# kkromberg/SpeechRecognition

Hardware: AMD Instinct MI355X
Metric: frames/sec scored+decoded (higher is better)
Workload: dtype f64

## Files before the change

include/srgpu.h:

```cpp
#ifndef SRGPU_H
#define SRGPU_H

#include <stddef.h>
#include <stdint.h>

#ifdef __cplusplus
extern "C" {
#endif

#if defined(__GNUC__)
#define SR_API __attribute__((visibility("default")))
#else
#define SR_API
#endif

#define SR_ABI_VERSION 4
SR_API int sr_abi_version(void);

#define SR_OK 0
#define SR_EINVAL (-1)
#define SR_EHIP (-2)
#define SR_ENODEV (-3)
#define SR_ELIMIT (-4)
#define SR_ENOMEM (-5)
// ... 205 lines not shown
                                         double* out_am);
SR_API int sr_bigram_lattice_nbest(uint32_t n_frames, uint64_t n_arcs, const uint32_t* word, const uint32_t* hist,
                                   const uint32_t* first, const uint32_t* last, const double* am, uint32_t n_words,
                                   uint32_t silence_word, const float* lm, double lm_scale, uint32_t n_best, uint32_t* out_words,
                                   uint64_t words_cap, uint64_t* out_off, double* out_cost, uint32_t* out_count);

typedef struct sr_bigram_stream sr_bigram_stream;
SR_API int sr_bigram_stream_open(sr_model* m, sr_bigram* b, const sr_bigram_params* p, uint32_t max_streams, uint64_t max_frames,
                                 sr_bigram_stream** out);
SR_API int sr_bigram_stream_begin(sr_bigram_stream* s, uint32_t* id);
SR_API int sr_bigram_stream_push(sr_bigram_stream* s, uint32_t n, const uint32_t* ids, const float* feats, const uint64_t* frame_off);
SR_API int sr_bigram_stream_partial(sr_bigram_stream* s, uint32_t id, uint32_t* out_word, float* out_score, uint32_t* out_time,
                                    uint32_t cap, uint32_t* count, uint64_t* frames);
SR_API int sr_bigram_stream_end(sr_bigram_stream* s, uint32_t id, uint32_t* out_word, float* out_score, uint32_t* out_time,
                                uint32_t cap, uint32_t* count);
SR_API int sr_bigram_stream_destroy(sr_bigram_stream* s);

SR_API int sr_probe_fp16_denormals(int device, int* preserved);
SR_API int sr_probe_fp16_accumulation(int device, int* within_model, double* worst_ratio);

typedef struct {
  double gmm_ms;
  uint64_t gmm_launches;
  double gmm_flops;
  double search_ms;
  uint64_t search_launches;
  double search_bytes;
  uint64_t frames;
  uint64_t refined_pairs;
  uint64_t refined_densities;
  double prefilter_ms;
  double refine_ms;
} sr_profile;
SR_API int sr_profile_enable(sr_model* m, int on);
SR_API int sr_profile_reset(sr_model* m);
SR_API int sr_profile_read(sr_model* m, sr_profile* out);

#ifdef __cplusplus
}
#endif
#endif
```

speechrecognition_amd/capi.py:

```python
from __future__ import annotations

import ctypes as C
import os

import numpy as np

HERE = os.path.dirname(os.path.abspath(__file__))
LIB_PATH = os.environ.get("SRGPU_LIB") or os.path.join(HERE, "libsrgpu.so")

GMM_MFMA, GMM_EXACT, GMM_PREFILTER, GMM_DEFAULT = 0, 1, 2, 3
POOL_GLOBAL, POOL_MIXTURE, POOL_NONE = 0, 1, 2
SEARCH_GENERAL_KERNEL = 1
SEARCH_SLOT_KERNEL = 2
BIGRAM_DENSE_STATES = 1
BIGRAM_GLOBAL_STATES = 2
SR_ECORRUPT = -7
SR_ABI_VERSION = 4

SYMBOLS = [
    "sr_abi_version", "sr_model_trim",
    "sr_last_error", "sr_device_count", "sr_model_create", "sr_model_load_mixset", "sr_model_destroy", "sr_model_info",
    "sr_corpus_upload", "sr_corpus_upload_async", "sr_corpus_wait", "sr_corpus_destroy", "sr_shard_utterances", "sr_recognize_batch_multi", "sr_score_corpus", "sr_score_frames", "sr_lexicon_create",
    "sr_lexicon_destroy", "sr_lexicon_describe", "sr_recognize_corpus", "sr_traceback_corpus", "sr_traceback_words", "sr_recognize_batch", "sr_align_corpus", "sr_align_corpus_pruned", "sr_path_scores_corpus", "sr_model_create_from_statistics", "sr_model_create_from_accumulated", "sr_mixset_write", "sr_model_set_tying", "sr_model_tying_info", "sr_model_topology", "sr_accumulate_corpus",
    "sr_state_posteriors_corpus", "sr_baum_welch_corpus", "sr_word_posteriors_corpus", "sr_recognize_confidence_corpus",
    "sr_net_occupancies_corpus", "sr_mmi_statistics_corpus", "sr_model_create_from_mmi_statistics",
    "sr_smbr_max_positions", "sr_net_accuracies_corpus", "sr_smbr_statistics_corpus",
    "sr_word_lattice_corpus", "sr_lattice_nbest",
    "sr_fmllr_statistics_corpus", "sr_fmllr_statistics_bw_corpus", "sr_fmllr_estimate", "sr_corpus_transform",
    "sr_bigram_create", "sr_bigram_destroy", "sr_bigram_describe", "sr_recognize_bigram_corpus",
    "sr_bigram_word_posteriors_corpus", "sr_recognize_bigram_confidence_corpus",
    "sr_bigram_occupancies_corpus", "sr_bigram_mmi_statistics_corpus",
    "sr_bigram_word_lattice_corpus", "sr_bigram_lattice_nbest",
    "sr_stream_open", "sr_stream_begin", "sr_stream_push", "sr_stream_partial", "sr_stream_end", "sr_stream_destroy",
    "sr_bigram_stream_open", "sr_bigram_stream_begin", "sr_bigram_stream_push", "sr_bigram_stream_partial", "sr_bigram_stream_end",
    "sr_bigram_stream_destroy",
    "sr_probe_fp16_denormals", "sr_probe_fp16_accumulation",
    "sr_profile_enable", "sr_profile_reset", "sr_profile_read",
]


class SrError(RuntimeError):
    def __init__(self, code, msg):
        super().__init__(f"libsrgpu error {code}: {msg}")
        self.code = code


def smbr_max_positions():
    n = C.c_uint32()
    _check(lib().sr_smbr_max_positions(C.byref(n)))
    return n.value


class SearchParams(C.Structure):
    _fields_ = [("am_threshold", C.c_double), ("word_penalty", C.c_double), ("gmm_kernel", C.c_int), ("flags", C.c_int)]


class BigramParams(C.Structure):
    _fields_ = [("acoustic_pruning", C.c_float), ("lm_pruning", C.c_float), ("gmm_kernel", C.c_int), ("max_word_ends", C.c_uint32), ("flags", C.c_int)]


class Profile(C.Structure):
    _fields_ = [("gmm_ms", C.c_double), ("gmm_launches", C.c_uint64), ("gmm_flops", C.c_double),
                ("search_ms", C.c_double), ("search_launches", C.c_uint64), ("search_bytes", C.c_double),
                ("frames", C.c_uint64), ("refined_pairs", C.c_uint64), ("refined_densities", C.c_uint64),
                ("prefilter_ms", C.c_double), ("refine_ms", C.c_double)]


_lib = None


# ... 48 lines not shown
        L.sr_recognize_confidence_corpus.argtypes = [vp, vp, vp, C.POINTER(SearchParams), dbl, vp, vp, vp, vp, vp]
        L.sr_net_occupancies_corpus.argtypes = [vp, vp, vp, C.POINTER(SearchParams), dbl, dbl, u32, vp, vp, vp, vp, vp, vp]
        L.sr_mmi_statistics_corpus.argtypes = [vp, vp, vp, C.POINTER(SearchParams), dbl, dbl, i32, vp, vp] + [vp] * 10
        L.sr_smbr_max_positions.argtypes = [vp]
        L.sr_net_accuracies_corpus.argtypes = [vp, vp, vp, C.POINTER(SearchParams), dbl, dbl, u32, vp, vp, vp, vp, vp, vp]
        L.sr_smbr_statistics_corpus.argtypes = [vp, vp, vp, C.POINTER(SearchParams), dbl, dbl, i32, vp] + [vp] * 10
        L.sr_model_create_from_mmi_statistics.argtypes = [vp] + [vp] * 8 + [dbl, dbl, dbl, C.POINTER(vp)]
        L.sr_word_lattice_corpus.argtypes = [vp, vp, vp, C.POINTER(SearchParams), dbl, u64, vp, vp, vp, vp, vp, vp, vp, vp]
        L.sr_lattice_nbest.argtypes = [u32, u64, vp, vp, vp, vp, u32, u32, vp, u64, vp, vp, C.POINTER(u32)]
        L.sr_bigram_create.argtypes = [vp, u32, vp, vp, u32, vp, vp, C.POINTER(vp)]
        L.sr_bigram_destroy.argtypes = [vp]
        L.sr_bigram_describe.argtypes = [vp, C.c_char_p, C.c_size_t]
        L.sr_recognize_bigram_corpus.argtypes = [vp, vp, vp, C.POINTER(BigramParams), vp, vp, vp, vp]
        L.sr_bigram_word_posteriors_corpus.argtypes = [vp, vp, vp, i32, dbl, dbl, u32, vp, vp, vp, vp]
        L.sr_bigram_occupancies_corpus.argtypes = [vp, vp, vp, i32, dbl, dbl, u32, vp, vp, vp, vp, vp, vp]
        L.sr_bigram_mmi_statistics_corpus.argtypes = [vp, vp, vp, i32, dbl, dbl, i32, vp, vp] + [vp] * 10
        L.sr_recognize_bigram_confidence_corpus.argtypes = [vp, vp, vp, C.POINTER(BigramParams), dbl, vp, vp, vp, vp, vp]
        L.sr_bigram_word_lattice_corpus.argtypes = [vp, vp, vp, i32, dbl, u64] + [vp] * 10
        L.sr_bigram_lattice_nbest.argtypes = [u32, u64, vp, vp, vp, vp, vp, u32, u32, vp, dbl, u32, vp, u64, vp, vp, C.POINTER(u32)]
        L.sr_stream_open.argtypes = [vp, vp, C.POINTER(SearchParams), u32, u64, C.POINTER(vp)]
        L.sr_stream_begin.argtypes = [vp, C.POINTER(u32)]
        L.sr_stream_push.argtypes = [vp, u32, vp, vp, vp]
        L.sr_stream_partial.argtypes = [vp, u32, vp, u32, C.POINTER(u32), C.POINTER(u64)]
        L.sr_stream_end.argtypes = [vp, u32, vp, u32, C.POINTER(u32), vp, vp, vp]
        L.sr_stream_destroy.argtypes = [vp]
        L.sr_bigram_stream_open.argtypes = [vp, vp, C.POINTER(BigramParams), u32, u64, C.POINTER(vp)]
        L.sr_bigram_stream_begin.argtypes = [vp, C.POINTER(u32)]
        L.sr_bigram_stream_push.argtypes = [vp, u32, vp, vp, vp]
        L.sr_bigram_stream_partial.argtypes = [vp, u32, vp, vp, vp, u32, C.POINTER(u32), C.POINTER(u64)]
        L.sr_bigram_stream_end.argtypes = [vp, u32, vp, vp, vp, u32, C.POINTER(u32)]
        L.sr_bigram_stream_destroy.argtypes = [vp]
        L.sr_probe_fp16_denormals.argtypes = [i32, C.POINTER(i32)]
        L.sr_probe_fp16_accumulation.argtypes = [i32, C.POINTER(i32), C.POINTER(dbl)]
        L.sr_profile_enable.argtypes = [vp, i32]
        L.sr_profile_reset.argtypes = [vp]
        L.sr_profile_read.argtypes = [vp, C.POINTER(Profile)]
        _lib = L
    return _lib


def _check(rc):
    if rc != 0:
        raise SrError(rc, lib().sr_last_error().decode(errors="replace"))


def device_count():
    n = C.c_int(0)
    _check(lib().sr_device_count(C.byref(n)))
    return n.value


def _ptr(a):
    return a.ctypes.data if a is not None else None


class Model:

    def __init__(self, handle):
        self.h = handle
        d, s, c = C.c_uint32(), C.c_uint32(), C.c_uint64()
        _check(lib().sr_model_info(self.h, C.byref(d), C.byref(s), C.byref(c)))
        self.dim, self.n_states, self.n_densities = d.value, s.value, c.value

    @classmethod
    def from_mixset(cls, path, dim, pooling=POOL_NONE, max_approx=True, device=0):
        h = C.c_void_p()
# ... 50 lines not shown
        self.close()

    def score_frames(self, feats, kernel=GMM_PREFILTER):
        feats = np.ascontiguousarray(feats, dtype=np.float32)
        out = np.empty((feats.shape[0], self.n_states), dtype=np.float64)
        _check(lib().sr_score_frames(self.h, _ptr(feats), feats.shape[0], kernel, _ptr(out)))
        return out

    def upload(self, feats, frame_off, asynchronous=False):
        return Corpus(self, feats, frame_off, asynchronous)

    def recognize_batch(self, lexicon, feats, frame_off, am_threshold, word_penalty, kernel=GMM_PREFILTER):
        feats = np.ascontiguousarray(feats, dtype=np.float32)
        frame_off = np.ascontiguousarray(frame_off, dtype=np.uint64)
        n = len(frame_off) - 1
        words = np.zeros(max(int(frame_off[-1]), 1), dtype=np.uint32)
        woff = np.zeros(n + 1, dtype=np.uint64)
        sp = SearchParams(am_threshold, word_penalty, kernel, 0)
        _check(lib().sr_recognize_batch(self.h, lexicon.h, C.byref(sp), _ptr(feats), _ptr(frame_off), n, _ptr(words), _ptr(woff)))
        return words[: int(woff[-1])].copy(), woff

    def lexicon(self, word_off, automaton, silence_idx, tdp, silence_state):
        return Lexicon(self, word_off, automaton, silence_idx, tdp, silence_state)

    def bigram(self, word_off, mixtures, silence_word, lm, tdp):
        return Bigram(self, word_off, mixtures, silence_word, lm, tdp)

    def stream(self, lexicon, am_threshold, word_penalty, kernel=GMM_PREFILTER, max_streams=1, max_frames=65535):
        return Stream(self, lexicon, am_threshold, word_penalty, kernel, max_streams, max_frames)

    def bigram_stream(self, bigram, acoustic_pruning=None, lm_pruning=None, kernel=GMM_PREFILTER, max_streams=1, max_frames=65535):
        return BigramStream(self, bigram, FLT_MAX if acoustic_pruning is None else acoustic_pruning,
                            FLT_MAX if lm_pruning is None else lm_pruning, kernel, max_streams, max_frames)

    def profile(self, on=True):
        _check(lib().sr_profile_enable(self.h, int(on)))
        _check(lib().sr_profile_reset(self.h))

    def profile_read(self):
        p = Profile()
        _check(lib().sr_profile_read(self.h, C.byref(p)))
        return {k: getattr(p, k) for k, _ in Profile._fields_}


FLT_MAX = float(np.finfo(np.float32).max)


class Bigram:

    def __init__(self, model, word_off, mixtures, silence_word, lm, tdp):
        self.model = model
        word_off = np.ascontiguousarray(word_off, dtype=np.uint32)
        mixtures = np.ascontiguousarray(mixtures, dtype=np.uint16)
        W = len(word_off) - 1
        lm = np.ascontiguousarray(lm, dtype=np.float32)
        assert lm.shape == (W, W)
        tdp = np.ascontiguousarray(tdp, dtype=np.float32)
        assert tdp.size == 8
        self.h = C.c_void_p()
        _check(lib().sr_bigram_create(model.h, W, _ptr(word_off), _ptr(mixtures), silence_word, _ptr(lm), _ptr(tdp), C.byref(self.h)))

    def describe(self):
        buf = C.create_string_buffer(32)
        _check(lib().sr_bigram_describe(self.h, buf, len(buf)))
        return buf.value.decode()

# ... 545 lines not shown
```

speechrecognition_amd/csrc/gmm_prefilter.hip:

```cpp
#include <hip/hip_runtime.h>
#include <stdint.h>

#include <algorithm>
#include <cmath>
#include <vector>

#include "kernels.h"

#ifndef SR_P16_NB
#define SR_P16_NB 4
#endif

namespace srgpu {

typedef float v4f __attribute__((ext_vector_type(4)));
static constexpr int kPWaves = 4;
static constexpr int kGroupBlocks = 8;

typedef _Float16 f16x8 __attribute__((ext_vector_type(8)));

__device__ inline uint32_t pack_f16x2(_Float16 l, _Float16 h) {
  return (uint32_t)__builtin_bit_cast(uint16_t, l) | ((uint32_t)__builtin_bit_cast(uint16_t, h) << 16);
}

// ... 286 lines not shown
  switch (ks32) {
    case 1: hipLaunchKernelGGL((gmm_prefilter16_kernel<1, SR_P16_NB>), grid, block, 0, stream, a); break;
    case 2: hipLaunchKernelGGL((gmm_prefilter16_kernel<2, SR_P16_NB>), grid, block, 0, stream, a); break;
    case 3: hipLaunchKernelGGL((gmm_prefilter16_kernel<3, SR_P16_NB>), grid, block, 0, stream, a); break;
    case 4: hipLaunchKernelGGL((gmm_prefilter16_kernel<4, SR_P16_NB>), grid, block, 0, stream, a); break;
    default: return hipErrorInvalidValue;
  }
  return hipGetLastError();
}
int gmm_prefilter_frames_per_tile() { return kPWaves * SR_P16_NB * 16; }

#pragma clang fp contract(off)

#ifndef SR_R_THREADS
#define SR_R_THREADS 768
#endif
#ifndef SR_R_BATCH
#define SR_R_BATCH 4
#endif
static constexpr int kRThreads = SR_R_THREADS;
static constexpr int kRThreadsWide = 512;
static constexpr int kRWaves = kRThreads / 64;
static constexpr int kRBatch = SR_R_BATCH;
#ifndef SR_R_BATCH_WIDE
#define SR_R_BATCH_WIDE 8
#endif
static constexpr int kRBatchWide = SR_R_BATCH_WIDE;
static constexpr uint32_t kRingEntries = 128;
static constexpr uint32_t kRingLists = 2 * 8 * kRingEntries;
static constexpr uint32_t kRingWave = 4 * kRingLists;
struct __attribute__((aligned(16))) RingEntry { uint32_t lf, mask; double score; };
struct __attribute__((packed, aligned(4))) RowPiece { float v[4]; };

template <int DT, int NS, int SPW, int CH, int NT = kRThreads, int VS = 1, bool DEFER = false>
__global__ __launch_bounds__(NT) void gmm_refine_kernel(GmmRefineArgs a) {
  static_assert(DT > 0 && (DT & 1), "padded dimension: odd");
  static_assert(!DEFER || CH > 1, "deferred lists: states of several chunks");
  constexpr int kRThreads = NT, kRWaves = NT / 64;
  static_assert(CH == 1 || CH == 2 || CH == 4, "chunks per state (half)");
  static_assert(VS == 1 || (VS == 2 && CH == 4), "two halves only of four-chunk states");
  static_assert(SPW % (CH * VS) == 0 && (CH == 1 || SPW % 4 == 0), "a state's chunks live in one workgroup");
  extern __shared__ __attribute__((aligned(1024))) unsigned char panel_raw[];
  const uint32_t D = (uint32_t)DT, tid = threadIdx.x;
  const int lane = tid & 63, wave = tid >> 6;
  const uint32_t s0 = blockIdx.x * SPW;
  const uint32_t ns = (s0 + SPW <= a.n_pstates) ? SPW : a.n_pstates - s0;
  const uint32_t state_bytes = (2u * D + 2u) * NS * 8u;
  const uint64_t f_begin = (uint64_t)blockIdx.y * a.frames_per_split;
  const uint64_t f_end = (f_begin + a.frames_per_split < a.n_frames) ? f_begin + a.frames_per_split : a.n_frames;

  {
    const uint32_t chunks = (ns * state_bytes + 1023u) >> 10;
    const unsigned char* src = reinterpret_cast<const unsigned char*>(a.rows) + (uint64_t)s0 * state_bytes + lane * 16;
    for (uint32_t ch = wave; ch < chunks; ch += kRWaves)
      __builtin_amdgcn_global_load_lds((const __attribute__((address_space(1))) void*)(src + (uint64_t)ch * 1024u),
                                       (__attribute__((address_space(3))) void*)(panel_raw + ch * 1024u), 16, 0, 0);
  }
  uint32_t nd[SPW];
#pragma unroll
  for (int j = 0; j < SPW; j++) nd[j] = (uint32_t)j < ns ? a.n_dens_ps[s0 + j] : 0u;
  __builtin_amdgcn_s_waitcnt(0x0F70);
  __syncthreads();
  if (f_begin >= f_end) return;

  uint32_t n_eval = 0;
  double x[DT];
  const __amdgpu_buffer_rsrc_t featsT_rsrc = __builtin_amdgcn_make_buffer_rsrc(
      const_cast<float*>(a.featsT), 0, (int)0xFFFFFFFFu, 0x00020000);
  const uint32_t ld4 = (uint32_t)a.n_frames_ld * 4u;
  auto load_x = [&](uint64_t f) __attribute__((always_inline)) {
    const uint32_t voff = (uint32_t)f * 4u;
#pragma unroll
    for (int k = 0; k < DT; k++)
      x[k] = (double)__builtin_bit_cast(float, __builtin_amdgcn_raw_buffer_load_b32(featsT_rsrc, voff, (uint32_t)k * ld4, 0));
  };
  auto load_x_row = [&](uint64_t f) __attribute__((always_inline)) {
    const float* xr = a.feats + f * (uint64_t)DT;
#pragma unroll
    for (int q = 0; q < DT / 4; q++) {
      const RowPiece t = reinterpret_cast<const RowPiece*>(xr)[q];
#pragma unroll
      for (int i = 0; i < 4; i++) x[4 * q + i] = (double)t.v[i];
    }
#pragma unroll
    for (int k = DT - DT % 4; k < DT; k++) x[k] = (double)xr[k];
  };
  auto evaluate = [&](const unsigned char* col0) __attribute__((always_inline)) -> double {
    const volatile __attribute__((address_space(3))) double* col =
        (const volatile __attribute__((address_space(3))) double*)col0;
    double l0 = 0.0, l1 = 0.0, dist, score;
    {
      constexpr int RB = NT == kRThreadsWide ? kRBatchWide : kRBatch;
      constexpr int NB_ = (DT + 1 + RB - 1) / RB;
      double pm[2][RB], pv[2][RB];
#pragma unroll
      for (int i = 0; i < RB; i++)
        if (i <= DT) { pm[0][i] = col[(2 * i) * NS]; pv[0][i] = col[(2 * i + 1) * NS]; }
#pragma unroll
      for (int b = 0; b < NB_; b++) {
        const int cur = b & 1;
        __builtin_amdgcn_sched_barrier(0);
#pragma unroll
// ... 2 lines not shown
          if (k <= DT) { pm[cur ^ 1][i] = col[(2 * k) * NS]; pv[cur ^ 1][i] = col[(2 * k + 1) * NS]; }
        }
        __builtin_amdgcn_sched_barrier(0);
#pragma unroll
        for (int i = 0; i < RB; i++) {
          const int k = b * RB + i;
          if (k < (int)(DT - (DT & 1))) {
            double u = x[k] - pm[cur][i];
            u = u * u;
            u = u * pv[cur][i];
            if (k & 1) l1 = l1 + u; else l0 = l0 + u;
          } else if (k == DT - 1) {
            dist = l0 + l1;
            const double t = x[k] - pm[cur][i];
            dist += t * t * pv[cur][i];
          } else if (k == DT) {
            if (!(DT & 1)) dist = l0 + l1;
            score = pm[cur][i] + dist / 2;
            score -= pv[cur][i];
          }
        }
        asm volatile("" : "+v"(l0), "+v"(l1));
      }
    }
    return score;
  };

  const double seed = 1e10;
  auto seeded_min = [&](double score) -> double {
    double r;
    asm("v_min_f64 %0, %1, %2" : "=v"(r) : "v"(score), "s"(seed));
    return r;
  };
  RingEntry* ring = reinterpret_cast<RingEntry*>(a.ring + ((uint64_t)(blockIdx.y * gridDim.x + blockIdx.x) * kRWaves + wave) * kRingWave);
  const bool counting = a.n_refined != nullptr;
  uint64_t cnt1 = 0, cnt2 = 0;
  const uint64_t wave_global = (uint64_t)(blockIdx.y * gridDim.x + blockIdx.x) * kRWaves + wave;
  RingEntry* seg = DEFER ? reinterpret_cast<RingEntry*>(a.defer) + wave_global * SPW * (uint64_t)a.defer_cap : nullptr;
  uint32_t dcnt[DEFER ? SPW : 1];
  if constexpr (DEFER) {
#pragma unroll
    for (int j = 0; j < SPW; j++) dcnt[j] = 0;
  }
  const uint64_t f_wave = f_begin + (uint64_t)wave * 64;
  auto frame_of = [&](uint32_t lf) -> uint64_t { return f_wave + (uint64_t)(lf >> 6) * kRThreads + (lf & 63u); };
  const uint32_t chunk_shift = CH == 1 ? (a.chunks == 1 ? 0u : a.chunks == 2 ? 1u : 2u) : CH == 2 ? 1u : VS == 2 ? 3u : 2u;

  const uint32_t n_it = (uint32_t)((f_end - f_begin + kRThreads - 1) / kRThreads);
  for (uint32_t it = 0; it < n_it; it++) {
    const uint64_t fr = f_wave + (uint64_t)it * kRThreads + lane;
    const bool valid = fr < f_end;
    const uint64_t f = valid ? fr : f_end - 1;
    const uint32_t lf = it * 64u + (uint32_t)lane;
    load_x(f);
    constexpr int RS = SPW / (CH * VS);
    double res[RS];
    if constexpr (CH == 1) {
#pragma unroll
      for (int h = 0; h < SPW / 4; h++) {
        const uint4 v = reinterpret_cast<const uint4*>(a.mask)[(uint64_t)((s0 >> 2) + h) * a.n_frames + f];
        const uint32_t mk[4] = {v.x, v.y, v.z, v.w};
#pragma unroll
        for (int jj = 0; jj < 4; jj++) {
          const int j = 4 * h + jj;
          const uint32_t n = nd[j];
          uint32_t mask = mk[jj];
          mask &= n >= 32 ? 0xFFFFFFFFu : ((1u << n) - 1u);
          res[j] = 1e10;
          if (n) {
            const double score = evaluate(panel_raw + (size_t)j * state_bytes + (uint32_t)__builtin_ctz(mask | 0x80000000u) * 8u);
// ... 394 lines not shown

hipError_t launch_transpose_feats(const float* feats, uint64_t n_frames, uint32_t dim, uint32_t dp, uint64_t ldT, float* out, float* featsP,
                                  hipStream_t stream) {
  if (n_frames == 0) return hipSuccess;
  if (dp < dim || (dp != dim && !featsP)) return hipErrorInvalidValue;
  hipLaunchKernelGGL(transpose_feats_kernel, dim3((unsigned)((n_frames + 63) / 64)), dim3(256), 0, stream, feats, n_frames, dim, dp, ldT, out,
                     dp != dim ? featsP : nullptr);
  return hipGetLastError();
}

int gmm_refine_slots(uint32_t max_dens, uint32_t padded_dim) { return padded_dim > 39 ? 32 : max_dens <= 8 ? 8 : max_dens <= 16 ? 16 : 32; }

uint32_t gmm_refine_padded_dim(uint32_t dim) {
  static const uint32_t bounds[] = {9, 17, 25, 33, 39, 47, 55, 63};
  const uint32_t need = dim | 1u;
  for (uint32_t b : bounds)
    if (need <= b) return b;
  return 0;
}

static int refine_threads(uint32_t dp) { return dp <= 47 ? kRThreads : kRThreadsWide; }
static int refine_spw(const GmmRefineArgs& a) {
  return (size_t)(2 * a.dim + 2) * a.n_slots * 8 * 8 <= 160 * 1024 ? 8 : 4;
}
static void refine_grid(const GmmRefineArgs& a, int spw, uint32_t* n_sgroups, uint64_t* splits, uint64_t* frames_per_split) {
  const uint64_t nt = (uint64_t)refine_threads(a.dim);
  *n_sgroups = (a.n_pstates + spw - 1) / spw;
  uint64_t sp = std::max<uint64_t>(1, (512 + *n_sgroups - 1) / *n_sgroups);
  sp = std::min<uint64_t>(sp, (a.n_frames + nt - 1) / nt);
  sp = std::max<uint64_t>(sp, 1);
  *frames_per_split = (a.n_frames + sp - 1) / sp;
  *splits = *frames_per_split ? (a.n_frames + *frames_per_split - 1) / *frames_per_split : 1;
}
size_t gmm_refine_ring_words(const GmmRefineArgs& a) {
  uint32_t g; uint64_t sp, fps;
  refine_grid(a, refine_spw(a), &g, &sp, &fps);
  return (size_t)g * sp * kRWaves * kRingWave;
}

static uint32_t defer_cap_for(const GmmRefineArgs& a, int spw) {
  uint32_t g; uint64_t sp, fps;
  refine_grid(a, spw, &g, &sp, &fps);
  const uint64_t per_wave = ((fps + kRThreads - 1) / kRThreads) * 64;
  return (uint32_t)std::min<uint64_t>(((per_wave / 4 + 63) & ~(uint64_t)63) + 64, 1u << 30);
}
void gmm_refine_defer_layout(const GmmRefineArgs& a, size_t budget_bytes, uint32_t cap_limit, uint32_t* cap, size_t* n_entries,
                             size_t* n_counts) {
  *cap = 0; *n_entries = 0; *n_counts = 0;
  if (a.chunks < 2 || a.dim > 39 || a.n_slots != 32 || a.n_frames == 0) return;
  uint32_t g; uint64_t sp, fps;
  refine_grid(a, 8, &g, &sp, &fps);
  uint32_t c = defer_cap_for(a, 8);
  if (cap_limit) c = std::min(c, cap_limit);
  const size_t segs = (size_t)g * sp * kRWaves * 8;
  if (segs * c * 16 > budget_bytes) return;
  *cap = c; *n_entries = segs * c; *n_counts = segs;
}

template <int DT, int NS, int SPW, int CH, int NT, int VS = 1>
static hipError_t launch_refine_one(const GmmRefineArgs& a0, hipStream_t stream) {
  GmmRefineArgs a = a0;
  const size_t state_bytes = (size_t)(2 * DT + 2) * NS * 8;
  const size_t smem = (SPW * state_bytes + 1023) & ~(size_t)1023;
  uint32_t n_sgroups;
  uint64_t splits;
  refine_grid(a, SPW, &n_sgroups, &splits, &a.frames_per_split);
  const dim3 grid(n_sgroups, (unsigned)splits), block(NT);
  if constexpr (CH > 1 && NT == kRThreads && SPW == 8) {
    if (a.defer && a.defer_cnt && a.defer_cap) {
      auto k1 = gmm_refine_kernel<DT, NS, SPW, CH, NT, VS, true>;
      auto k2 = gmm_drain_kernel<DT, NS, SPW, CH, NT, VS>;
      hipError_t e = hipFuncSetAttribute((const void*)k1, hipFuncAttributeMaxDynamicSharedMemorySize, (int)smem);
      if (e == hipSuccess) e = hipFuncSetAttribute((const void*)k2, hipFuncAttributeMaxDynamicSharedMemorySize, (int)smem);
      if (e != hipSuccess) return e;
      hipLaunchKernelGGL(k1, grid, block, smem, stream, a);
      if ((e = hipGetLastError()) != hipSuccess) return e;
      hipLaunchKernelGGL(k2, grid, block, smem, stream, a);
      return hipGetLastError();
    }
  }
  a.defer = nullptr; a.defer_cnt = nullptr; a.defer_cap = 0;
  auto kernel = gmm_refine_kernel<DT, NS, SPW, CH, NT, VS>;
  hipError_t e = hipFuncSetAttribute((const void*)kernel, hipFuncAttributeMaxDynamicSharedMemorySize, (int)smem);
  if (e != hipSuccess) return e;
  hipLaunchKernelGGL(kernel, grid, block, smem, stream, a);
  return hipGetLastError();
}

template <int DT>
static hipError_t launch_refine_narrow(const GmmRefineArgs& a, hipStream_t stream) {
  switch (a.n_slots) {
    case 8: return launch_refine_one<DT, 8, 8, 1, kRThreads>(a, stream);
    case 16: return launch_refine_one<DT, 16, 8, 1, kRThreads>(a, stream);
    case 32:
      if (a.chunks == 2) return launch_refine_one<DT, 32, 8, 2, kRThreads>(a, stream);
      if (a.chunks == 4) return launch_refine_one<DT, 32, 8, 4, kRThreads>(a, stream);
      if (a.chunks == 8) return launch_refine_one<DT, 32, 8, 4, kRThreads, 2>(a, stream);
      return launch_refine_one<DT, 32, 8, 1, kRThreads>(a, stream);
    default: return hipErrorInvalidValue;
  }
}
template <int DT>
static hipError_t launch_refine_wide(const GmmRefineArgs& a, hipStream_t stream) {
  if (a.n_slots != 32) return hipErrorInvalidValue;
  if (a.chunks == 2) return launch_refine_one<DT, 32, 4, 2, kRThreadsWide>(a, stream);
  if (a.chunks == 4) return launch_refine_one<DT, 32, 4, 4, kRThreadsWide>(a, stream);
  return launch_refine_one<DT, 32, 4, 1, kRThreadsWide>(a, stream);
}

hipError_t launch_gmm_refine(const GmmRefineArgs& a, hipStream_t stream) {
  if (a.n_frames == 0) return hipSuccess;
  if (!a.ring || (uint64_t)a.dim * a.n_frames_ld * 4u >= (1ull << 32)) return hipErrorInvalidValue;
  if (a.chunks != 1 && (a.n_slots != 32 || (a.chunks != 2 && a.chunks != 4 && a.chunks != 8))) return hipErrorInvalidValue;
  if (a.chunks == 8 && a.dim > 39) return hipErrorInvalidValue;
// ... 18 lines not shown
```

speechrecognition_amd/csrc/handles.h:

```cpp
#pragma once
#include <hip/hip_runtime.h>

#include <atomic>
#include <condition_variable>
#include <cstdint>
#include <map>
#include <memory>
#include <mutex>
#include <string>
#include <thread>
#include <vector>

#include "../../include/srgpu.h"
#include "host_util.h"
#include "kernels.h"

namespace srhost {
int fail(int code, const char* fmt, ...) __attribute__((format(printf, 2, 3)));
}

#define HIP_TRY(expr)                                                                             \
  do {                                                                                            \
    hipError_t e_ = (expr);                                                                       \
    if (e_ != hipSuccess) return srhost::fail(SR_EHIP, "%s: %s (%s:%d)", #expr, hipGetErrorString(e_), __FILE__, __LINE__); \
// ... 57 lines not shown
  int ksteps = 0;
  uint32_t n_blocks = 0, n_groups = 0;
  DevBuf<double> apack;
  DevBuf<uint32_t> blk_meta, grp_state;
  std::vector<uint32_t> group_first_block;
  std::map<uint32_t, std::unique_ptr<DevBuf<uint32_t>>> split_tabs, pf_split_tabs;
  const uint32_t *split_cur = nullptr, *pf_split_cur = nullptr;
  uint32_t split_ny = 0;
  int pf_ks32 = 0;
  uint32_t pf_groups = 0, pf_ny = 0, max_dens = 0, pf_slots = 0, pf_chunks = 1, pf_pstates = 0;
  DevBuf<unsigned char> pf_apack;
  DevBuf<float> pf_lim, featsT, featsP;
  DevBuf<uint4> pf_defer;
  DevBuf<uint32_t> pf_defer_cnt;
  int neg_possible = -1;
  uint32_t pf_dp = 0;
  DevBuf<uint32_t> pf_mask, pf_ndens, pf_ring;
  DevBuf<double> pf_rows;
  DevBuf<unsigned long long> pf_counter;
  hipStream_t s_copy = nullptr;
  float* staging[2] = {nullptr, nullptr};
  hipEvent_t staging_free[2] = {nullptr, nullptr};
  std::atomic<bool> staging_busy{false};
  std::mutex spare_mu;
  std::unique_ptr<CorpusSpare> spare;
  std::vector<sr_corpus*> corpora;
  hipStream_t s_gmm = nullptr, s_search = nullptr;
  DevBuf<double> scores[2];
  hipEvent_t ev_scored[2] = {nullptr, nullptr}, ev_consumed[2] = {nullptr, nullptr};
  size_t chunk_frames = 0;
  bool overlap = true;
  size_t defer_budget = (size_t)32 << 30;
  uint32_t defer_cap_limit = 0;
  size_t fb_budget = (size_t)1 << 30;
  bool profiling = false;
  std::vector<EventPair> events;
  sr_profile prof{};
};

struct sr_corpus {
  sr_model* model = nullptr;
  sr_feeder* feeder = nullptr;
  uint32_t n_utts = 0;
  uint64_t n_frames = 0;
  std::vector<uint64_t> frame_off;
  DevBuf<float> feats;
  DevBuf<uint64_t> d_frame_off;
  DevBuf<uint32_t> utt_order;
  size_t order_chunk_frames = 0;
  DevBuf<double> tb_score;
  DevBuf<uint16_t> tb_word, tb_bkp;
  DevBuf<uint32_t> out_words, out_count, out_flags;
  DevBuf<unsigned char> big_ws;
  DevBuf<uint16_t> automata, out_states;
  DevBuf<uint64_t> aut_off, bp_off, al_blk_frame0;
  DevBuf<uint32_t> al_list_off, al_states, al_blk_frames, al_blk_list;
  DevBuf<uint8_t> backptr;
  DevBuf<double> out_cost, path_scores;
  DevBuf<uint64_t> pair_off;
  DevBuf<uint32_t> pair_frame, key_mean, key_var, iota, keys_sorted, pairs_sorted, row_begin;
  DevBuf<double> pair_w, acc_mean, acc_var, w_mean, w_var;
  bool acc_valid = false;
  uint32_t acc_n_mean = 0, acc_n_var = 0;
  DevBuf<unsigned char> sort_temp;
  DevBuf<double> fb_trellis, fb_item_w, fb_weight;
  DevBuf<uint64_t> fb_trellis_off, fb_pair_cnt, fb_pair_end;
// ... 140 lines not shown
```

speechrecognition_amd/csrc/kernels.h:

```cpp
#pragma once
#include <hip/hip_runtime.h>
#include <stdint.h>

#include <vector>

namespace srgpu {

struct GmmMfmaArgs {
  const float* feats;
  uint64_t n_frames;
  uint32_t dim;
  const double* apack;
  const uint32_t* blk_meta;
  const uint32_t* grp_state;
  const uint32_t* split_begin;
  double* out;
  uint32_t ld;
  uint32_t nx, ny;
};
int gmm_mfma_ksteps_for_dim(uint32_t dim);
int gmm_mfma_frames_per_tile(int ksteps);
hipError_t launch_gmm_mfma(const GmmMfmaArgs& a, int ksteps, bool sum, hipStream_t stream);

struct GmmExactArgs {
// ... 25 lines not shown

struct GmmPrefilterArgs {
  const float* feats;
  uint64_t n_frames;
  uint32_t dim;
  const unsigned char* apack;
  const float* grp_lim;
  const uint32_t* split_begin;
  uint32_t* mask;
  uint32_t nx, ny;
  uint32_t chunks;
};
struct PfBound { float kappa, acc, abs, sub; };
constexpr float kPfRes16 = 4.8835e-4f;
inline constexpr PfBound pf_bound(int ks32) {
  return ks32 == 4 ? PfBound{1.05e-3f, 1.6e-5f, 7.0e-7f, 3.38e-7f} : PfBound{1.05e-3f, 1.1e-5f, 6.0e-7f, 2.92e-7f};
}
struct GmmRefineArgs {
  const float* feats;
  const float* featsT;
  uint64_t n_frames, n_frames_ld;
  uint32_t dim, n_pstates, chunks;
  const uint32_t* n_dens_ps;
  const double* rows;
  uint32_t n_slots;
  const uint32_t* mask;
  double* out; uint32_t ld;
  uint64_t frames_per_split;
  unsigned long long* n_refined;
  uint32_t* ring;
  void* defer;
  uint32_t* defer_cnt;
  uint32_t defer_cap;
};
void gmm_refine_defer_layout(const GmmRefineArgs& a, size_t budget_bytes, uint32_t cap_limit, uint32_t* cap, size_t* n_entries,
                             size_t* n_counts);
size_t gmm_refine_ring_words(const GmmRefineArgs& a);
hipError_t launch_gmm_prefilter(const GmmPrefilterArgs& a, int ks32, hipStream_t stream);
int gmm_prefilter_frames_per_tile();
hipError_t probe_fp16_denormals(hipStream_t stream, bool* preserved);
hipError_t probe_fp16_accumulation(hipStream_t stream, int ks32, bool* ok, double* worst_ratio);
uint32_t gmm_refine_padded_dim(uint32_t dim);
int gmm_refine_slots(uint32_t max_dens, uint32_t padded_dim);
hipError_t launch_gmm_refine(const GmmRefineArgs& a, hipStream_t stream);
hipError_t launch_transpose_feats(const float* feats, uint64_t n_frames, uint32_t dim, uint32_t dp, uint64_t ldT, float* out, float* featsP,
                                  hipStream_t stream);

struct DecodeNet {
  uint32_t n_slots;
  uint32_t n_words;
  const uint32_t* slot_info;
  const uint32_t* slot_word;
  const uint32_t* word_end_slot;
  uint32_t silence_word;
  double tdp_loop, tdp_forward, tdp_skip;
  uint32_t silence_state;
};
static constexpr uint32_t kSlotPos0 = 1u << 16;
static constexpr uint32_t kSlotPos1 = 1u << 17;
static constexpr uint32_t kSlotEnd = 1u << 18;
static constexpr uint32_t kSlotSilState = 1u << 19;
static constexpr uint32_t kSlotSilWord = 1u << 20;
static constexpr uint32_t kSlotFirstSil = 1u << 21;
static constexpr uint32_t kSlotSingle = 1u << 22;
struct FastNet {
  uint32_t n_slots;
// ... 511 lines not shown
```

speechrecognition_amd/csrc/srgpu_api.cpp:

```cpp
#include <hip/hip_runtime.h>

#include <algorithm>
#include <cmath>
#include <cstdarg>
#include <cstdio>
#include <cstdlib>
#include <cstring>
#include <limits>
#include <map>
#include <memory>
#include <mutex>
#include <numeric>
#include <queue>
#include <set>
#include <string>
#include <vector>

#include "../../include/srgpu.h"
#include "host_util.h"
#include "kernels.h"
#include "traceback.h"

using namespace srgpu;
using srhost::guarded;
// ... 293 lines not shown
    std::unique_ptr<DevBuf<uint32_t>> fresh(new DevBuf<uint32_t>());
    HIP_TRY(fresh->upload(sb.data(), sb.size()));
    it = m->split_tabs.insert_or_assign(ny, std::move(fresh)).first;
  }
  m->split_cur = it->second->p;
  m->split_ny = ny;
  return SR_OK;
}

int prof_begin(sr_model* m, hipStream_t s, int kind, EventPair* ep) {
  if (!m->profiling) return SR_OK;
  ep->kind = kind;
  HIP_TRY(hipEventCreate(&ep->a));
  HIP_TRY(hipEventCreate(&ep->b));
  HIP_TRY(hipEventRecord(ep->a, s));
  return SR_OK;
}
int prof_end(sr_model* m, hipStream_t s, EventPair* ep) {
  if (!m->profiling) return SR_OK;
  HIP_TRY(hipEventRecord(ep->b, s));
  m->events.push_back(*ep);
  return SR_OK;
}

int resolve_dense_kernel(const sr_model* m, int gmm_kernel) {
  if (gmm_kernel == SR_GMM_DEFAULT) gmm_kernel = m->max_approx ? SR_GMM_PREFILTER : SR_GMM_MFMA;
  if (gmm_kernel == SR_GMM_MFMA && m->ksteps == 0) gmm_kernel = SR_GMM_EXACT;
  return gmm_kernel;
}

GmmRefineArgs refine_shape(const sr_model* m, uint64_t n_frames) {
  GmmRefineArgs ra{};
  ra.n_frames = n_frames; ra.dim = m->pf_dp; ra.n_pstates = m->pf_pstates; ra.n_slots = m->pf_slots; ra.chunks = m->pf_chunks;
  return ra;
}
struct DeferLayout { uint32_t cap; size_t n_e, n_c; };
DeferLayout defer_layout(const sr_model* m, uint64_t n_frames) {
  DeferLayout d;
  gmm_refine_defer_layout(refine_shape(m, n_frames), m->defer_budget, m->defer_cap_limit, &d.cap, &d.n_e, &d.n_c);
  return d;
}

int reserve_scoring(sr_model* m, int gmm_kernel, uint64_t n_max) {
  gmm_kernel = resolve_dense_kernel(m, gmm_kernel);
  if ((gmm_kernel == SR_GMM_MFMA && !m->mfma_packed) || (gmm_kernel == SR_GMM_PREFILTER && !m->pf_packed)) {
    int rc = srhost::ensure_host_tables(m);
    if (rc) return rc;
  }
  if (gmm_kernel == SR_GMM_MFMA && !m->mfma_packed) {
    int rc = pack_model(m, m->h_dens_off.data(), m->h_means.data(), m->h_inv_vars.data(), m->h_norm.data(), m->h_logw.data());
    if (rc) return rc;
    m->mfma_packed = true;
  }
  if (gmm_kernel == SR_GMM_PREFILTER && !m->pf_packed) {
    int rc = pack_prefilter(m, m->h_dens_off.data(), m->h_means.data(), m->h_inv_vars.data(), m->h_norm.data(), m->h_logw.data());
    if (rc) return rc;
    m->pf_packed = true;
  }
  if (gmm_kernel == SR_GMM_PREFILTER && m->pf_ks32 > 0 && n_max > 0) {
    const uint64_t ldT = (n_max + 63) & ~(uint64_t)63;
    const size_t want_T = (size_t)ldT * m->pf_dp, want_mask = (size_t)((m->pf_groups + 1u) & ~1u) * n_max * 4;
    const size_t want_P = m->pf_dp != m->dim ? (size_t)n_max * m->pf_dp + 4 : 0;
    const size_t want_ring = gmm_refine_ring_words(refine_shape(m, n_max));
    if (want_T > m->featsT.n || want_P > m->featsP.n || want_mask > m->pf_mask.n || want_ring > m->pf_ring.n) HIP_TRY(hipStreamSynchronize(m->s_gmm));
    HIP_TRY(m->featsT.ensure(want_T));
    if (want_P) HIP_TRY(m->featsP.ensure(want_P));
// ... 283 lines not shown
  if (e != hipSuccess) { *count = 0; return fail(SR_ENODEV, "hipGetDeviceCount: %s", hipGetErrorString(e)); }
  *count = n;
  return SR_OK;
  });
}

}

namespace srhost {

int model_shell(int device, uint32_t dim, uint32_t n_states, const uint32_t* dens_off, int max_approx, sr_model** out) {
  *out = nullptr;
  if (!dens_off) return fail(SR_EINVAL, "null model table");
  if (dim == 0 || n_states == 0) return fail(SR_EINVAL, "dim and n_states must be positive");
  const int ks = gmm_mfma_ksteps_for_dim(dim);
  if (dim > 160) return fail(SR_ELIMIT, "dim %u unsupported (max 160: the exact kernel keeps a workgroup's frames in LDS)", dim);
  if (dens_off[0] != 0) return fail(SR_EINVAL, "dens_off[0] must be 0");
  for (uint32_t s = 0; s < n_states; s++)
    if (dens_off[s + 1] < dens_off[s]) return fail(SR_EINVAL, "dens_off must be non-decreasing (state %u)", s);
  const uint64_t C = dens_off[n_states];
  if (C >= (1ull << 31)) return fail(SR_ELIMIT, "too many densities");
  int ndev = 0;
  if (hipGetDeviceCount(&ndev) != hipSuccess || ndev == 0) return fail(SR_ENODEV, "no HIP device visible");
  if (device < 0 || device >= ndev) return fail(SR_EINVAL, "device %d out of range (0..%d)", device, ndev - 1);
  hipDeviceProp_t prop;
  HIP_TRY(hipGetDeviceProperties(&prop, device));
  if (strncmp(prop.gcnArchName, "gfx950", 6) != 0)
    return fail(SR_ENODEV, "device %d is %s; libsrgpu is built for gfx950 (MI355X) only", device, prop.gcnArchName);
  HIP_TRY(hipSetDevice(device));
  sr_model* m = new sr_model();
  std::unique_ptr<sr_model, int (*)(sr_model*)> own(m, sr_model_destroy);
  m->device = device; m->dim = dim; m->n_states = n_states; m->n_dens = C; m->max_approx = max_approx != 0;
  m->ksteps = ks;
  m->ld = (n_states + 7u) & ~7u;
  hipError_t e;
  if ((e = hipStreamCreateWithFlags(&m->s_gmm, hipStreamNonBlocking)) != hipSuccess ||
      (e = hipStreamCreateWithFlags(&m->s_search, hipStreamNonBlocking)) != hipSuccess)
    return fail(SR_EHIP, "hipStreamCreate: %s", hipGetErrorString(e));
  for (int i = 0; i < 2; i++)
    if ((e = hipEventCreateWithFlags(&m->ev_scored[i], hipEventDisableTiming)) != hipSuccess ||
        (e = hipEventCreateWithFlags(&m->ev_consumed[i], hipEventDisableTiming)) != hipSuccess)
      return fail(SR_EHIP, "hipEventCreate: %s", hipGetErrorString(e));
  if ((e = m->dens_off.upload(dens_off, n_states + 1)) != hipSuccess) return fail(SR_EHIP, "model upload: %s", hipGetErrorString(e));
  uint32_t mx = 0;
  for (uint32_t s = 0; s < n_states; s++) mx = std::max(mx, dens_off[s + 1] - dens_off[s]);
  m->max_dens = std::max(1u, mx);
  m->h_dens_off.assign(dens_off, dens_off + n_states + 1);
  const char* env = getenv("SRGPU_SCORE_CHUNK_MB");
  size_t chunk_bytes = (size_t)49152 << 20;
  {
    size_t free_b = 0, total_b = 0;
    if (hipMemGetInfo(&free_b, &total_b) == hipSuccess && total_b) chunk_bytes = std::min(chunk_bytes, total_b / 6);
  }
  if (env) chunk_bytes = (size_t)atol(env) << 20;
  m->chunk_frames = std::max<size_t>(1, chunk_bytes / ((size_t)m->ld * sizeof(double)));
  m->chunk_frames = std::min<size_t>(m->chunk_frames, ((size_t)1 << 32) / (4 * (size_t)dim) - 128);
  if (const char* ov = getenv("SRGPU_OVERLAP")) m->overlap = atoi(ov) != 0;
  if (const char* e = getenv("SRGPU_DEFER_MB")) m->defer_budget = (size_t)strtoull(e, nullptr, 10) << 20;
  if (const char* e = getenv("SRGPU_FB_MB")) m->fb_budget = std::max<size_t>(1, (size_t)strtoull(e, nullptr, 10)) << 20;
  if (const char* e = getenv("SRGPU_DEFER_CAP")) m->defer_cap_limit = std::max(1u, (uint32_t)strtoul(e, nullptr, 10));
  *out = own.release();
  return SR_OK;
}

int ensure_host_tables(sr_model* m) {
  const size_t C = m->n_dens, D = m->dim;
// ... 3208 lines not shown

int sr_bigram_stream_end(sr_bigram_stream* s, uint32_t id, uint32_t* out_word, float* out_score, uint32_t* out_time, uint32_t cap,
                         uint32_t* count) {
  return guarded(__func__, [&]() -> int {
  if (!s || !count || ((!out_word || !out_score || !out_time) && cap)) return fail(SR_EINVAL, "null argument");
  const int64_t slot = s->slots.find(id);
  if (slot < 0) return fail(SR_EINVAL, "stream id %u is not open", id);
  int rc = check_model(s->model);
  if (rc) return rc;
  rc = bigram_stream_items(s, (uint32_t)slot, id, out_word, out_score, out_time, cap, count);
  if (rc == SR_EINVAL) return rc;
  s->slots.open[slot] = 0;
  return rc;
  });
}

int sr_bigram_stream_destroy(sr_bigram_stream* s) {
  return guarded(__func__, [&]() -> int {
  if (!s) return SR_OK;
  if (s->model) { (void)hipSetDevice(s->model->device); (void)hipDeviceSynchronize(); }
  delete s;
  return SR_OK;
  });
}

int sr_profile_enable(sr_model* m, int on) {
  return guarded(__func__, [&]() -> int {
  if (!m) return fail(SR_EINVAL, "null model handle");
  m->profiling = on != 0;
  return SR_OK;
  });
}

int sr_profile_reset(sr_model* m) {
  return guarded(__func__, [&]() -> int {
  int rc = check_model(m);
  if (rc) return rc;
  HIP_TRY(hipDeviceSynchronize());
  for (auto& ep : m->events) { (void)hipEventDestroy(ep.a); (void)hipEventDestroy(ep.b); }
  m->events.clear();
  m->prof = sr_profile{};
  HIP_TRY(m->pf_counter.ensure(1));
  HIP_TRY(hipMemset(m->pf_counter.p, 0, sizeof(unsigned long long)));
  return SR_OK;
  });
}

int sr_profile_read(sr_model* m, sr_profile* out) {
  return guarded(__func__, [&]() -> int {
  int rc = check_model(m);
  if (rc) return rc;
  if (!out) return fail(SR_EINVAL, "out is null");
  HIP_TRY(hipDeviceSynchronize());
  for (auto& ep : m->events) {
    float ms = 0.f;
    HIP_TRY(hipEventElapsedTime(&ms, ep.a, ep.b));
    if (ep.kind == 0) { m->prof.gmm_ms += ms; m->prof.gmm_launches++; }
    else if (ep.kind == 1) { m->prof.search_ms += ms; m->prof.search_launches++; }
    else if (ep.kind == 2) m->prof.prefilter_ms += ms;
    else m->prof.refine_ms += ms;
    (void)hipEventDestroy(ep.a);
    (void)hipEventDestroy(ep.b);
  }
  m->events.clear();
  if (m->pf_counter.p) {
    unsigned long long n = 0;
// ... 10 lines not shown
```

Baseline: 13.48 million.

## Balance GMM refine work evenly across one workgroup per CU

Adds a persistent-style refine kernel that launches one workgroup per compute unit. It divides the state-group × frame-block work units evenly among those workgroups, with each workgroup iterating over contiguous segments. The goal is to remove load imbalance and tail effects of the fixed 2D grid of state groups by frame splits. The trade-off is fewer resident workgroups for latency hiding, plus extra syncs between segments. A test hook to override the workgroup count is also added.

```diff
diff --git a/include/srgpu.h b/include/srgpu.h
--- a/include/srgpu.h
+++ b/include/srgpu.h
@@ -261,6 +261,7 @@
   double prefilter_ms;
   double refine_ms;
 } sr_profile;
+SR_API int sr_test_refine_workgroups(sr_model* m, uint32_t n_workgroups);
 SR_API int sr_profile_enable(sr_model* m, int on);
 SR_API int sr_profile_reset(sr_model* m);
 SR_API int sr_profile_read(sr_model* m, sr_profile* out);
diff --git a/speechrecognition_amd/capi.py b/speechrecognition_amd/capi.py
--- a/speechrecognition_amd/capi.py
+++ b/speechrecognition_amd/capi.py
@@ -35,7 +35,7 @@
     "sr_bigram_stream_open", "sr_bigram_stream_begin", "sr_bigram_stream_push", "sr_bigram_stream_partial", "sr_bigram_stream_end",
     "sr_bigram_stream_destroy",
     "sr_probe_fp16_denormals", "sr_probe_fp16_accumulation",
-    "sr_profile_enable", "sr_profile_reset", "sr_profile_read",
+    "sr_test_refine_workgroups", "sr_profile_enable", "sr_profile_reset", "sr_profile_read",
 ]
 
 
@@ -150,6 +150,7 @@
         L.sr_bigram_stream_destroy.argtypes = [vp]
         L.sr_probe_fp16_denormals.argtypes = [i32, C.POINTER(i32)]
         L.sr_probe_fp16_accumulation.argtypes = [i32, C.POINTER(i32), C.POINTER(dbl)]
+        L.sr_test_refine_workgroups.argtypes = [vp, u32]
         L.sr_profile_enable.argtypes = [vp, i32]
         L.sr_profile_reset.argtypes = [vp]
         L.sr_profile_read.argtypes = [vp, C.POINTER(Profile)]
@@ -266,6 +267,9 @@
     def bigram_stream(self, bigram, acoustic_pruning=None, lm_pruning=None, kernel=GMM_PREFILTER, max_streams=1, max_frames=65535):
         return BigramStream(self, bigram, FLT_MAX if acoustic_pruning is None else acoustic_pruning,
                             FLT_MAX if lm_pruning is None else lm_pruning, kernel, max_streams, max_frames)
+
+    def test_refine_workgroups(self, n):
+        _check(lib().sr_test_refine_workgroups(self.h, int(n)))
 
     def profile(self, on=True):
         _check(lib().sr_profile_enable(self.h, int(on)))
diff --git a/speechrecognition_amd/csrc/gmm_prefilter.hip b/speechrecognition_amd/csrc/gmm_prefilter.hip
--- a/speechrecognition_amd/csrc/gmm_prefilter.hip
+++ b/speechrecognition_amd/csrc/gmm_prefilter.hip
@@ -342,8 +342,35 @@
 struct __attribute__((aligned(16))) RingEntry { uint32_t lf, mask; double score; };
 struct __attribute__((packed, aligned(4))) RowPiece { float v[4]; };
 
+template <int DT, int NS, int SPW, int CH, int NT, int VS, bool DEFER, bool EVEN>
+__device__ __forceinline__ void refine_segment(const GmmRefineArgs& a, uint32_t sgroup, uint64_t f_begin, uint64_t f_end, uint32_t wg);
+
 template <int DT, int NS, int SPW, int CH, int NT = kRThreads, int VS = 1, bool DEFER = false>
 __global__ __launch_bounds__(NT) void gmm_refine_kernel(GmmRefineArgs a) {
+  const uint64_t f_begin = (uint64_t)blockIdx.y * a.frames_per_split;
+  const uint64_t f_end = (f_begin + a.frames_per_split < a.n_frames) ? f_begin + a.frames_per_split : a.n_frames;
+  refine_segment<DT, NS, SPW, CH, NT, VS, DEFER, false>(a, blockIdx.x, f_begin, f_end, blockIdx.y * gridDim.x + blockIdx.x);
+}
+
+template <int DT, int NS, int SPW, int NT>
+__global__ __launch_bounds__(NT) void gmm_refine_kernel_even(GmmRefineArgs a) {
+  const uint32_t W = ((a.n_pstates + SPW - 1) / SPW) * a.its_per_group;
+  uint32_t unit = blockIdx.x * W / gridDim.x;
+  const uint32_t unit_end = (blockIdx.x + 1) * W / gridDim.x;
+  while (unit < unit_end) {
+    const uint32_t ipg = a.its_per_group;
+    const uint32_t g = unit / ipg, it_begin = unit - g * ipg;
+    const uint32_t n = (ipg - it_begin < unit_end - unit) ? ipg - it_begin : unit_end - unit;
+    const uint64_t f_begin = (uint64_t)it_begin * NT, f_stop = (uint64_t)(it_begin + n) * NT;
+    refine_segment<DT, NS, SPW, 1, NT, 1, false, true>(a, g, f_begin, f_stop < a.n_frames ? f_stop : a.n_frames, blockIdx.x);
+    unit += n;
+    if (unit < unit_end) __syncthreads();
+  }
+}
+
+template <int DT, int NS, int SPW, int CH, int NT, int VS, bool DEFER, bool EVEN>
+__device__ __forceinline__ void refine_segment(const GmmRefineArgs& a, const uint32_t sgroup, const uint64_t f_begin, const uint64_t f_end,
+                                               const uint32_t wg) {
   static_assert(DT > 0 && (DT & 1), "padded dimension: odd");
   static_assert(!DEFER || CH > 1, "deferred lists: states of several chunks");
   constexpr int kRThreads = NT, kRWaves = NT / 64;
@@ -353,11 +380,9 @@
   extern __shared__ __attribute__((aligned(1024))) unsigned char panel_raw[];
   const uint32_t D = (uint32_t)DT, tid = threadIdx.x;
   const int lane = tid & 63, wave = tid >> 6;
-  const uint32_t s0 = blockIdx.x * SPW;
+  const uint32_t s0 = sgroup * SPW;
   const uint32_t ns = (s0 + SPW <= a.n_pstates) ? SPW : a.n_pstates - s0;
   const uint32_t state_bytes = (2u * D + 2u) * NS * 8u;
-  const uint64_t f_begin = (uint64_t)blockIdx.y * a.frames_per_split;
-  const uint64_t f_end = (f_begin + a.frames_per_split < a.n_frames) ? f_begin + a.frames_per_split : a.n_frames;
 
   {
     const uint32_t chunks = (ns * state_bytes + 1023u) >> 10;
@@ -377,7 +402,8 @@
   double x[DT];
   const __amdgpu_buffer_rsrc_t featsT_rsrc = __builtin_amdgcn_make_buffer_rsrc(
       const_cast<float*>(a.featsT), 0, (int)0xFFFFFFFFu, 0x00020000);
-  const uint32_t ld4 = (uint32_t)a.n_frames_ld * 4u;
+  uint32_t ld4 = (uint32_t)a.n_frames_ld * 4u;
+  if constexpr (EVEN) asm volatile("" : "+s"(ld4));
   auto load_x = [&](uint64_t f) __attribute__((always_inline)) {
     const uint32_t voff = (uint32_t)f * 4u;
 #pragma unroll
@@ -446,10 +472,10 @@
     asm("v_min_f64 %0, %1, %2" : "=v"(r) : "v"(score), "s"(seed));
     return r;
   };
-  RingEntry* ring = reinterpret_cast<RingEntry*>(a.ring + ((uint64_t)(blockIdx.y * gridDim.x + blockIdx.x) * kRWaves + wave) * kRingWave);
+  RingEntry* ring = reinterpret_cast<RingEntry*>(a.ring + ((uint64_t)wg * kRWaves + wave) * kRingWave);
   const bool counting = a.n_refined != nullptr;
   uint64_t cnt1 = 0, cnt2 = 0;
-  const uint64_t wave_global = (uint64_t)(blockIdx.y * gridDim.x + blockIdx.x) * kRWaves + wave;
+  const uint64_t wave_global = (uint64_t)wg * kRWaves + wave;
   RingEntry* seg = DEFER ? reinterpret_cast<RingEntry*>(a.defer) + wave_global * SPW * (uint64_t)a.defer_cap : nullptr;
   uint32_t dcnt[DEFER ? SPW : 1];
   if constexpr (DEFER) {
@@ -910,10 +936,15 @@
   *frames_per_split = (a.n_frames + sp - 1) / sp;
   *splits = *frames_per_split ? (a.n_frames + *frames_per_split - 1) / *frames_per_split : 1;
 }
+static bool refine_even(const GmmRefineArgs& a) {
+  if (a.n_wg == 0 || a.chunks != 1 || refine_spw(a) != 8 || refine_threads(a.dim) != kRThreads) return false;
+  const uint64_t W = (uint64_t)((a.n_pstates + 7) / 8) * ((a.n_frames + kRThreads - 1) / kRThreads);
+  return W <= 0xFFFFFFFFull / a.n_wg;
+}
 size_t gmm_refine_ring_words(const GmmRefineArgs& a) {
   uint32_t g; uint64_t sp, fps;
   refine_grid(a, refine_spw(a), &g, &sp, &fps);
-  return (size_t)g * sp * kRWaves * kRingWave;
+  return (size_t)std::max<uint64_t>(g * sp, a.n_wg) * kRWaves * kRingWave;
 }
 
 static uint32_t defer_cap_for(const GmmRefineArgs& a, int spw) {
@@ -958,6 +989,16 @@
     }
   }
   a.defer = nullptr; a.defer_cnt = nullptr; a.defer_cap = 0;
+  if constexpr (CH == 1 && VS == 1 && NT == kRThreads && SPW == 8) {
+    if (refine_even(a)) {
+      a.its_per_group = (uint32_t)((a.n_frames + NT - 1) / NT);
+      auto even = gmm_refine_kernel_even<DT, NS, SPW, NT>;
+      hipError_t e = hipFuncSetAttribute((const void*)even, hipFuncAttributeMaxDynamicSharedMemorySize, (int)smem);
+      if (e != hipSuccess) return e;
+      hipLaunchKernelGGL(even, dim3(a.n_wg), block, smem, stream, a);
+      return hipGetLastError();
+    }
+  }
   auto kernel = gmm_refine_kernel<DT, NS, SPW, CH, NT, VS>;
   hipError_t e = hipFuncSetAttribute((const void*)kernel, hipFuncAttributeMaxDynamicSharedMemorySize, (int)smem);
   if (e != hipSuccess) return e;
diff --git a/speechrecognition_amd/csrc/handles.h b/speechrecognition_amd/csrc/handles.h
--- a/speechrecognition_amd/csrc/handles.h
+++ b/speechrecognition_amd/csrc/handles.h
@@ -113,6 +113,8 @@
   bool overlap = true;
   size_t defer_budget = (size_t)32 << 30;
   uint32_t defer_cap_limit = 0;
+  uint32_t n_cus = 0;
+  uint32_t refine_wgs = 0;
   size_t fb_budget = (size_t)1 << 30;
   bool profiling = false;
   std::vector<EventPair> events;
diff --git a/speechrecognition_amd/csrc/kernels.h b/speechrecognition_amd/csrc/kernels.h
--- a/speechrecognition_amd/csrc/kernels.h
+++ b/speechrecognition_amd/csrc/kernels.h
@@ -81,6 +81,8 @@
   void* defer;
   uint32_t* defer_cnt;
   uint32_t defer_cap;
+  uint32_t n_wg;
+  uint32_t its_per_group;
 };
 void gmm_refine_defer_layout(const GmmRefineArgs& a, size_t budget_bytes, uint32_t cap_limit, uint32_t* cap, size_t* n_entries,
                              size_t* n_counts);
diff --git a/speechrecognition_amd/csrc/srgpu_api.cpp b/speechrecognition_amd/csrc/srgpu_api.cpp
--- a/speechrecognition_amd/csrc/srgpu_api.cpp
+++ b/speechrecognition_amd/csrc/srgpu_api.cpp
@@ -349,6 +349,7 @@
 GmmRefineArgs refine_shape(const sr_model* m, uint64_t n_frames) {
   GmmRefineArgs ra{};
   ra.n_frames = n_frames; ra.dim = m->pf_dp; ra.n_pstates = m->pf_pstates; ra.n_slots = m->pf_slots; ra.chunks = m->pf_chunks;
+  ra.n_wg = m->refine_wgs ? m->refine_wgs : m->n_cus;
   return ra;
 }
 struct DeferLayout { uint32_t cap; size_t n_e, n_c; };
@@ -698,6 +699,7 @@
   std::unique_ptr<sr_model, int (*)(sr_model*)> own(m, sr_model_destroy);
   m->device = device; m->dim = dim; m->n_states = n_states; m->n_dens = C; m->max_approx = max_approx != 0;
   m->ksteps = ks;
+  m->n_cus = (uint32_t)std::max(1, prop.multiProcessorCount);
   m->ld = (n_states + 7u) & ~7u;
   hipError_t e;
   if ((e = hipStreamCreateWithFlags(&m->s_gmm, hipStreamNonBlocking)) != hipSuccess ||
@@ -3972,6 +3974,17 @@
   });
 }
 
+int sr_test_refine_workgroups(sr_model* m, uint32_t n_workgroups) {
+  return guarded(__func__, [&]() -> int {
+  int rc = check_model(m);
+  if (rc) return rc;
+  if (n_workgroups > 65536u) return fail(SR_EINVAL, "n_workgroups %u: at most 65536", n_workgroups);
+  HIP_TRY(hipStreamSynchronize(m->s_gmm));
+  m->refine_wgs = n_workgroups;
+  return SR_OK;
+  });
+}
+
 int sr_profile_reset(sr_model* m) {
   return guarded(__func__, [&]() -> int {
   int rc = check_model(m);
```

Result: no change. 13.47 million (-0.0%).
